# lucidrains/se3-transformer-pytorch

Hardware: NVIDIA H100
Metric: point-clouds/sec fwd (higher is better)
Workload: dtype f32

## Files before the change

### se3_transformer_pytorch_b200/csrc/zgemm.cu

```cuda
#include "common.cuh"
#include "tc_ptx.cuh"
#include <algorithm>
#include <cstdlib>
#include <type_traits>

namespace se3 {

constexpr int kZThreads = 384;
constexpr int kZMaxSeg = 16;
constexpr uint32_t kZWRingBytes = 196608;

template <int V>
using ic = std::integral_constant<int, V>;

template <class F, int... I>
__device__ __forceinline__ void static_for_seq(F&& f, std::integer_sequence<int, I...>) {
  (f(ic<I>()), ...);
}
template <int N, class F>
__device__ __forceinline__ void static_for(F&& f) {
  static_for_seq(f, std::make_integer_sequence<int, N>());
}

struct ZSeg {
  const float* U;
  const float* X;
  int Ci, ncomp, cplus, cminus, n_stage, pad;
};

struct ZParams {
  ZSeg seg[kZMaxSeg];
  int n_seg;
  const uint8_t* w_img;
  const float* sx;
  float* out;
  int64_t E;
  int64_t out_es;
  int comp_off[2];
  int n_mt, n_nt, S, flush_stages;
};

__device__ __forceinline__ void z_frag(const float (&v)[2][4], uint32_t (&hi)[4], uint32_t (&lo)[4]) {
  split_h2(v[0][0], v[0][1], hi[0], lo[0]);
  split_h2(v[1][0], v[1][1], hi[1], lo[1]);
  split_h2(v[0][2], v[0][3], hi[2], lo[2]);
  split_h2(v[1][2], v[1][3], hi[3], lo[3]);
}

template <int NR>
__device__ __forceinline__ void z_mma3(float (&d)[NR], const uint32_t (&hi)[4], const uint32_t (&lo)[4], uint64_t b_hi, uint64_t b_lo,
                                       uint32_t scale_d = 1) {
  if constexpr (NR == 64) {
    wgmma_rs_n128(d, hi, b_hi, scale_d);
    wgmma_rs_n128(d, lo, b_hi);
    wgmma_rs_n128(d, hi, b_lo);
  } else {
    wgmma_rs_n64(d, hi, b_hi, scale_d);
    wgmma_rs_n64(d, lo, b_hi);
    wgmma_rs_n64(d, hi, b_lo);
  }
}

template <int MODE, int N, int NC>
__global__ void __launch_bounds__(kZThreads, 1)
zgemm_kernel(const __grid_constant__ ZParams prm) {
  static_assert((MODE == 1 || MODE == 4) ? NC == 128 : NC == 64, "CTA width");
  static_assert(N % NC == 0 && (MODE == 1 || N == 128), "weight image tile");
  constexpr int NA = (MODE == 3) ? 3 : (MODE == 2) ? 2 : 1;
  constexpr int NO = (MODE == 2 || MODE == 3) ? 2 : 1;
  constexpr int NR = NC / 2;
  constexpr int NH = N / NC;
  constexpr uint32_t kImgStage = 2u * N * 128u;
  constexpr uint32_t kStageBytes = 2u * NC * 128u;
  constexpr int WS = (kZWRingBytes / kStageBytes > 8) ? 8 : (int)(kZWRingBytes / kStageBytes);

  extern __shared__ uint8_t smem_raw[];
  const uint32_t raw = smem_u32(smem_raw);
  const uint32_t base = (raw + 1023u) & ~1023u;
  const uint32_t sW = base;
  const uint32_t bar_w_full = sW + WS * kStageBytes;
  const uint32_t bar_w_empty = bar_w_full + 8 * WS;

  const int warp = __shfl_sync(0xffffffffu, (int)(threadIdx.x >> 5), 0), lane = threadIdx.x & 31;
  const int S = prm.S, FS = prm.flush_stages;
  const int n_ct = prm.n_nt * NH;
  const int ctile = (int)(blockIdx.x % n_ct);
  const int64_t mt = blockIdx.x / n_ct;
  const int nt = ctile / NH, hs = ctile % NH;

  if (threadIdx.x == 0) {
    for (int s = 0; s < WS; ++s) {
      mbar_init(bar_w_full + 8 * s, 1);
      mbar_init(bar_w_empty + 8 * s, 8);
    }
    asm volatile("fence.mbarrier_init.release.cluster;" ::: "memory");
  }
  __syncthreads();

  if (warp < 4) {
    asm volatile("setmaxnreg.dec.sync.aligned.u32 40;");
    if (warp == 0 && lane == 0) {
      const uint8_t* wsrc = prm.w_img + (size_t)nt * S * kImgStage + (size_t)hs * NC * 128u;
      for (int s = 0; s < S; ++s) {
        const int slot = s % WS;
        mbar_wait(bar_w_empty + 8 * slot, ((uint32_t)(s / WS) & 1u) ^ 1u);
        mbar_arrive_expect_tx(bar_w_full + 8 * slot, kStageBytes);
        bulk_g2s(sW + slot * kStageBytes, wsrc + (size_t)s * kImgStage, NC * 128u, bar_w_full + 8 * slot);
        bulk_g2s(sW + slot * kStageBytes + NC * 128u, wsrc + (size_t)s * kImgStage + N * 128u, NC * 128u, bar_w_full + 8 * slot);
      }
    }
    return;
  }
  asm volatile("setmaxnreg.inc.sync.aligned.u32 232;");
  const int ct = threadIdx.x - 128;
  const int r0 = (ct >> 7) * 64 + ((ct >> 5) & 3) * 16 + (lane >> 2);
  const int kq = 2 * (lane & 3);
  int64_t eg[2];
  bool live[2];
  float sxe[2];
#pragma unroll
  for (int rs = 0; rs < 2; ++rs) {
    eg[rs] = mt * SE3_TILE_E + r0 + 8 * rs;
    live[rs] = eg[rs] < prm.E;
    sxe[rs] = (live[rs] && MODE != 4) ? prm.sx[eg[rs]] : 1.f;
  }
  float D[NA][NR], acc[NO][NR];
#pragma unroll
  for (int a = 0; a < NA; ++a)
#pragma unroll
    for (int j = 0; j < NR; ++j) D[a][j] = 0.f;
#pragma unroll
  for (int a = 0; a < NO; ++a)
#pragma unroll
    for (int j = 0; j < NR; ++j) acc[a][j] = 0.f;
  int blk_start = 0;
  int fresh = 0;

  auto release = [&](int s) {
    __syncwarp();
    if (lane == 0) mbar_arrive(bar_w_empty + 8 * (s % WS));
  };
  auto drain_after = [&](int s) { return s + 1 == S || s + 1 - blk_start == FS; };
  auto drain = [&](int s) {
#pragma unroll
    for (int j = 0; j < NR; ++j) {
      if (MODE == 3) {
        acc[0][j] += D[0][j] - D[NA - 1][j];
        acc[1][j] += D[0][j] + D[NA > 1 ? 1 : 0][j];
      } else {
#pragma unroll
        for (int a = 0; a < NA; ++a) acc[a][j] += D[a][j];
      }
      if (MODE == 2 || MODE == 4)
#pragma unroll
        for (int a = 0; a < NA; ++a) D[a][j] = 0.f;
    }
    fresh = (1 << NA) - 1;
    blk_start = s + 1;
  };
  auto finish_stage = [&](int s) {
    wgmma_commit();
    wgmma_wait0();
    release(s);
    if (drain_after(s)) drain(s);
  };

  constexpr int ZR = (MODE == 3) ? 2 : 4;
  float u[2][4];
  auto zf = [&](const float (&y)[2], uint32_t (&hi)[4], uint32_t (&lo)[4]) {
    float v[2][4];
#pragma unroll
    for (int rs = 0; rs < 2; ++rs)
#pragma unroll
      for (int q = 0; q < 4; ++q) v[rs][q] = u[rs][q] * y[rs];
    z_frag(v, hi, lo);
  };
  auto chunk_mma = [&](auto cc, auto ac, int s, const float (&y)[2], uint64_t b_hi, uint64_t b_lo) {
    constexpr int C = decltype(cc)::value, A = decltype(ac)::value;
    wgmma_wait<ZR - 1>();
    if (C == ZR - 1 && s != blk_start) release(s - 1);
    uint32_t hi[4], lo[4];
    zf(y, hi, lo);
    wgmma_fence();
    z_mma3<NR>(D[A], hi, lo, b_hi + 2 * C, b_lo + 2 * C, ((fresh >> A) & 1) ^ 1);
    fresh &= ~(1 << A);
    wgmma_commit();
  };
  auto end_stage = [&](int s) {
    if (drain_after(s)) {
      wgmma_wait0();
      release(s);
      drain(s);
    }
  };
  auto wait_stage = [&](int s, uint64_t& b_hi, uint64_t& b_lo) {
    mbar_wait(bar_w_full + 8 * (s % WS), (uint32_t)(s / WS) & 1u);
    const uint32_t wb = sW + (uint32_t)(s % WS) * kStageBytes;
    b_hi = wg_desc_sw128(wb);
    b_lo = wg_desc_sw128(wb + NC * 128u);
  };

  if constexpr (MODE == 4) {
    const ZSeg& z = prm.seg[0];
    const int M = z.ncomp, Dn = z.Ci;
    int64_t node[2];
    int m[2];
    float sc[2];
    const float* xrow[2];
#pragma unroll
    for (int rs = 0; rs < 2; ++rs) {
      node[rs] = live[rs] ? eg[rs] / M : 0;
      m[rs] = live[rs] ? (int)(eg[rs] - node[rs] * M) : 0;
      sc[rs] = live[rs] ? prm.sx[node[rs]] : 1.f;
      xrow[rs] = z.X + ((size_t)node[rs] * Dn) * M + m[rs];
    }
    for (int s = 0; s < S; ++s) {
      float v[4][2][4];
#pragma unroll
      for (int c = 0; c < 4; ++c)
#pragma unroll
        for (int rs = 0; rs < 2; ++rs)
#pragma unroll
          for (int q = 0; q < 4; ++q) {
            const int d = 64 * s + 16 * c + kq + (q & 1) + 8 * (q >> 1);
            v[c][rs][q] = live[rs] ? __ldg(xrow[rs] + (size_t)d * M) * sc[rs] : 0.f;
          }
      uint64_t b_hi, b_lo;
      wait_stage(s, b_hi, b_lo);
      uint32_t hi[4][4], lo[4][4];
#pragma unroll
      for (int c = 0; c < 4; ++c) z_frag(v[c], hi[c], lo[c]);
      wgmma_fence();
#pragma unroll
      for (int c = 0; c < 4; ++c) z_mma3<NR>(D[0], hi[c], lo[c], b_hi + 2 * c, b_lo + 2 * c);
      finish_stage(s);
    }
#pragma unroll
    for (int rs = 0; rs < 2; ++rs) {
      if (!live[rs]) continue;
      const float inv = 1.f / sc[rs];
      const int64_t Eo = prm.out_es;
      const size_t o0 = (size_t)nt * N + (size_t)hs * NC + kq;
      float* dst = prm.out + ((size_t)node[rs] * Eo + o0) * M + m[rs];
      const float* res = z.U ? z.U + ((size_t)node[rs] * Eo + o0) * M + m[rs] : nullptr;
#pragma unroll
      for (int g = 0; g < NC / 8; ++g)
#pragma unroll
        for (int b = 0; b < 2; ++b) {
          const size_t o = (size_t)(8 * g + b) * M;
          dst[o] = acc[0][4 * g + 2 * rs + b] * inv + (res ? __ldg(res + o) : 0.f);
        }
    }
  } else {
    int s = 0;
    for (int sg = 0; sg < prm.n_seg; ++sg) {
      const ZSeg& z = prm.seg[sg];
      const int ns = z.n_stage;
      const size_t istride = (size_t)z.ncomp * 128;
      const float* xp = z.X + ((size_t)mt * z.Ci * z.ncomp + z.cplus) * 128 + r0;
      const float* xm = z.X + ((size_t)mt * z.Ci * z.ncomp + z.cminus) * 128 + r0;
#pragma unroll
      for (int rs = 0; rs < 2; ++rs) {
        const float* urow = z.U + (size_t)(live[rs] ? eg[rs] : 0) * 64;
#pragma unroll
        for (int q = 0; q < 4; ++q) u[rs][q] = live[rs] ? __ldg(urow + kq + (q & 1) + 8 * (q >> 1)) * sxe[rs] : 0.f;
      }
      if constexpr (MODE == 1) {
        float y[4][2];
#pragma unroll
        for (int c = 0; c < 4; ++c)
#pragma unroll
          for (int rs = 0; rs < 2; ++rs) y[c][rs] = __ldg(xp + c * istride + 8 * rs);
#pragma unroll 1
        for (int sl = 0; sl < ns; ++sl, ++s) {
          const float* xn = (sl + 1 < ns) ? xp + 4 * istride : xp;
          uint64_t b_hi, b_lo;
          wait_stage(s, b_hi, b_lo);
          static_for<4>([&](auto cc) {
            constexpr int C = decltype(cc)::value;
            chunk_mma(cc, ic<0>(), s, y[C], b_hi, b_lo);
#pragma unroll
            for (int rs = 0; rs < 2; ++rs) y[C][rs] = __ldg(xn + C * istride + 8 * rs);
          });
          end_stage(s);
          xp = xn;
        }
      } else if constexpr (MODE == 2) {
#pragma unroll 1
        for (int sl = 0; sl < ns; ++sl, ++s) {
          float yp[2][2], ym[2][2];
#pragma unroll
          for (int il = 0; il < 2; ++il)
#pragma unroll
            for (int rs = 0; rs < 2; ++rs) {
              const size_t o = (size_t)(2 * sl + il) * istride + 8 * rs;
              yp[il][rs] = __ldg(xp + o);
              ym[il][rs] = __ldg(xm + o);
            }
          uint64_t b_hi, b_lo;
          wait_stage(s, b_hi, b_lo);
          uint32_t hp[2][4], lp[2][4], hm[2][4], lm[2][4];
#pragma unroll
          for (int il = 0; il < 2; ++il) {
            zf(yp[il], hp[il], lp[il]);
            zf(ym[il], hm[il], lm[il]);
          }
          uint32_t hn[2][4], ln[2][4];
#pragma unroll
          for (int il = 0; il < 2; ++il)
#pragma unroll
            for (int q = 0; q < 4; ++q) { hn[il][q] = hm[il][q] ^ 0x80008000u; ln[il][q] = lm[il][q] ^ 0x80008000u; }
          wgmma_fence();
#pragma unroll
          for (int il = 0; il < 2; ++il) {
            const uint64_t ba_hi = b_hi + 2 * (2 * il), ba_lo = b_lo + 2 * (2 * il);
            const uint64_t bb_hi = b_hi + 2 * (2 * il + 1), bb_lo = b_lo + 2 * (2 * il + 1);
            z_mma3<NR>(D[0], hp[il], lp[il], ba_hi, ba_lo);
            z_mma3<NR>(D[0], hn[il], ln[il], bb_hi, bb_lo);
            z_mma3<NR>(D[NA - 1], hm[il], lm[il], ba_hi, ba_lo);
            z_mma3<NR>(D[NA - 1], hp[il], lp[il], bb_hi, bb_lo);
          }
          finish_stage(s);
        }
      } else {
        const int dmo = (z.cminus - z.cplus) * 128;
        float x[4][2][2];
#pragma unroll
        for (int j = 0; j < 4; ++j)
#pragma unroll
          for (int rs = 0; rs < 2; ++rs) {
            x[j][0][rs] = __ldg(xp + j * istride + 8 * rs);
            x[j][1][rs] = __ldg(xp + dmo + j * istride + 8 * rs);
          }
        const int np = ns / 3;
#pragma unroll 1
        for (int p = 0; p < np; ++p) {
          const size_t adv = (p + 1 < np) ? 4 * istride : 0;
          static_for<3>([&](auto tc) {
            uint64_t b_hi, b_lo;
            wait_stage(s, b_hi, b_lo);
            static_for<4>([&](auto cc) {
              constexpr int Q = 4 * decltype(tc)::value + decltype(cc)::value, J = Q / 3, T = Q % 3;
              float y[2];
#pragma unroll
              for (int rs = 0; rs < 2; ++rs) {
                const float cp = x[J][0][rs], dm = x[J][1][rs];
                y[rs] = (T == 0) ? cp : (T == 1) ? (dm - cp) : (cp + dm);
              }
              chunk_mma(cc, ic<T>(), s, y, b_hi, b_lo);
              if constexpr (T == 2) {
#pragma unroll
                for (int rs = 0; rs < 2; ++rs) {
                  x[J][0][rs] = __ldg(xp + adv + J * istride + 8 * rs);
                  x[J][1][rs] = __ldg(xp + adv + dmo + J * istride + 8 * rs);
                }
              }
            });
            end_stage(s);
            ++s;
          });
          xp += adv;
        }
      }
    }

#pragma unroll
    for (int rs = 0; rs < 2; ++rs) {
      if (!live[rs]) continue;
      const float inv = 1.f / sxe[rs];
#pragma unroll
      for (int a = 0; a < NO; ++a) {
        float* dst = prm.out + (size_t)eg[rs] * prm.out_es + prm.comp_off[a] + (size_t)nt * N + (size_t)hs * NC + kq;
#pragma unroll
        for (int g = 0; g < NC / 8; ++g)
          *reinterpret_cast<float2*>(dst + 8 * g) = make_float2(acc[a][4 * g + 2 * rs] * inv, acc[a][4 * g + 2 * rs + 1] * inv);
      }
    }
  }
}

__global__ void zpack_kernel(const float* __restrict__ Fp, int Kp, int col0, int Co, int CiF, int N, int S, int stage0, int n_stage,
                             int gauss, uint8_t* __restrict__ img) {
  const int nt = blockIdx.y, sl = blockIdx.x;
  uint8_t* dst = img + ((size_t)nt * S + stage0 + sl) * (2u * N * 128u);
  for (int t = threadIdx.x; t < N * 64; t += blockDim.x) {
    const int r = t >> 6, k = t & 63;
    const int o = nt * N + r;
    float w = 0.f;
    if (gauss) {
      const int q = sl * 4 + (k >> 4);
      const int ty = q % 3, i = q / 3;
      if (2 * i + 1 < CiF && o < Co) {
        const float wa = Fp[((size_t)o * CiF + 2 * i) * Kp + col0 + (k & 15)], wb = Fp[((size_t)o * CiF + 2 * i + 1) * Kp + col0 + (k & 15)];
        w = (ty == 0) ? wa + wb : (ty == 1) ? wa : wb;
      }
    } else {
      const int c = sl * 4 + (k >> 4);
      if (c < CiF && o < Co) w = Fp[((size_t)o * CiF + c) * Kp + col0 + (k & 15)];
    }
    const __half hi = __float2half_rn(w);
    const __half lo = __float2half_rn(w - __half2float(hi));
    const uint32_t off = (uint32_t)(r * 128 + (((k >> 3) ^ (r & 7)) << 4) + (k & 7) * 2);
    *reinterpret_cast<__half*>(dst + off) = hi;
    *reinterpret_cast<__half*>(dst + (size_t)N * 128 + off) = lo;
  }
}

template <int MODE, int N, int NC>
static int launch_z(const ZParams& prm, cudaStream_t s) {
  constexpr uint32_t kStageBytes = 2u * NC * 128u;
  constexpr int WS = (kZWRingBytes / kStageBytes > 8) ? 8 : (int)(kZWRingBytes / kStageBytes);
  const size_t smem = 1024 + (size_t)WS * kStageBytes + 256;
  auto kern = zgemm_kernel<MODE, N, NC>;
  SE3_CUDA_OK(cudaFuncSetAttribute(kern, cudaFuncAttributeMaxDynamicSharedMemorySize, (int)smem));
  const int64_t grid = (int64_t)prm.n_mt * prm.n_nt * (N / NC);
  SE3_REQUIRE(grid < 2147483647ll, "se3_zgemm: grid too large");
  kern<<<(unsigned)grid, kZThreads, smem, s>>>(prm);
  SE3_LAUNCH_OK();
  return SE3_OK;
}

static int z_env_int(const char* name, int dflt) {
  const char* v = getenv(name);
  return v ? atoi(v) : dflt;
}

}

extern "C" int se3_zgemm_tile_n(int Co, int mode) {
  if (Co <= 0 || Co % 128 != 0) return -1;
  if (mode == 2 || mode == 3 || mode == 4) return 128;
  if (mode != 1) return -1;
  return (Co % 256 == 0) ? 256 : 128;
}

extern "C" int64_t se3_zgemm_image_bytes(int Co, int mode, int total_stages) {
  const int N = se3_zgemm_tile_n(Co, mode);
  if (N < 0 || total_stages <= 0) return -1;
  return (int64_t)(Co / N) * total_stages * 2 * N * 128;
}

extern "C" int se3_zgemm_pack(const float* Fp, int Kp, int col0, int Co, int CiF, int mode, int total_stages, int stage0, void* image,
                              void* stream) {
  using namespace se3;
  const int N = se3_zgemm_tile_n(Co, mode);
  SE3_REQUIRE(N > 0, "se3_zgemm_pack: Co=%d must be a multiple of 128 (mode %d)", Co, mode);
  SE3_REQUIRE(Fp != nullptr && image != nullptr, "se3_zgemm_pack: null pointer");
  SE3_REQUIRE(Kp >= 16 && Kp % 16 == 0 && col0 >= 0 && col0 + 16 <= Kp, "se3_zgemm_pack: bad column range");
  SE3_REQUIRE(CiF > 0 && (mode == 1 || CiF % 2 == 0), "se3_zgemm_pack: bad sizes");
  const int n_stage = (mode == 3) ? 3 * (int)ceil_div(CiF / 2, 4) : (int)ceil_div(CiF, 4);
  SE3_REQUIRE(stage0 >= 0 && stage0 + n_stage <= total_stages, "se3_zgemm_pack: stage range outside the image");
  zpack_kernel<<<dim3((unsigned)n_stage, (unsigned)(Co / N)), 256, 0, as_stream(stream)>>>(Fp, Kp, col0, Co, CiF, N, total_stages, stage0, n_stage,
                                                                                         mode == 3 ? 1 : 0, reinterpret_cast<uint8_t*>(image));
  SE3_LAUNCH_OK();
  return SE3_OK;
}

extern "C" int se3_linear_tc_fwd(const float* x, const void* w_img, const float* res, const float* sx, int64_t nodes, int D, int Eo,
                                 int M, float* out, void* stream) {
  using namespace se3;
  SE3_REQUIRE(nodes > 0 && M >= 1 && M <= 11, "se3_linear_tc_fwd: bad sizes");
  SE3_REQUIRE(D > 0 && D % 64 == 0 && Eo > 0 && Eo % 128 == 0, "se3_linear_tc_fwd: D=%d must be a multiple of 64 and Eo=%d of 128", D, Eo);
  SE3_REQUIRE(x != nullptr && w_img != nullptr && sx != nullptr && out != nullptr, "se3_linear_tc_fwd: null pointer");
  ZParams prm;
  prm.n_seg = 1;
  prm.seg[0].U = res;
  prm.seg[0].X = x;
  prm.seg[0].Ci = D;
  prm.seg[0].ncomp = M;
  prm.seg[0].cplus = prm.seg[0].cminus = 0;
  prm.seg[0].n_stage = D / 64;
  prm.seg[0].pad = 0;
  prm.w_img = reinterpret_cast<const uint8_t*>(w_img);
  prm.sx = sx;
  prm.out = out;
  prm.E = nodes * M;
  prm.out_es = Eo;
  prm.comp_off[0] = prm.comp_off[1] = 0;
  prm.n_mt = (int)ceil_div(prm.E, SE3_TILE_E);
  prm.n_nt = Eo / 128;
  prm.S = D / 64;
  prm.flush_stages = std::max(1, z_env_int("SE3B200_Z_FLUSH", 8));
  return launch_z<4, 128, 128>(prm, as_stream(stream));
}

extern "C" int se3_zgemm_fwd(const se3_zseg* segs, int n_seg, const void* w_img, const float* sx, int64_t E, int Co, int mode,
                             float* out, int64_t out_edge_stride, int comp_off0, int comp_off1, int flush_stages, void* stream) {
  using namespace se3;
  const int N = se3_zgemm_tile_n(Co, mode);
  SE3_REQUIRE(N > 0 && mode != 4, "se3_zgemm_fwd: Co=%d must be a multiple of 128 and mode 1, 2 or 3 (got %d)", Co, mode);
  SE3_REQUIRE(E > 0 && n_seg >= 1 && n_seg <= kZMaxSeg, "se3_zgemm_fwd: bad sizes (1..%d segments)", kZMaxSeg);
  SE3_REQUIRE(segs != nullptr && w_img != nullptr && sx != nullptr && out != nullptr, "se3_zgemm_fwd: null pointer");
  SE3_REQUIRE(out_edge_stride >= Co && out_edge_stride % 4 == 0 && comp_off0 % 4 == 0 && comp_off1 % 4 == 0 &&
              (reinterpret_cast<uintptr_t>(out) & 15) == 0, "se3_zgemm_fwd: output rows must be 16-byte aligned");
  ZParams prm;
  prm.n_seg = n_seg;
  int S = 0;
  const int F = (mode == 1) ? 1 : 2;
  for (int i = 0; i < n_seg; ++i) {
    const se3_zseg& z = segs[i];
    SE3_REQUIRE(z.U != nullptr && z.X != nullptr && z.Ci > 0 && z.ncomp >= 1 && z.cplus >= 0 && z.cplus < z.ncomp &&
                z.cminus >= 0 && z.cminus < z.ncomp, "se3_zgemm_fwd: bad segment %d", i);
    SE3_REQUIRE((z.Ci * F) % 4 == 0 && (mode != 3 || z.Ci % 4 == 0), "se3_zgemm_fwd: C_in * F = %d must be a multiple of 4 (mode 3: C_in % 4 == 0)", z.Ci * F);
    prm.seg[i].U = z.U;
    prm.seg[i].X = z.X;
    prm.seg[i].Ci = z.Ci;
    prm.seg[i].ncomp = z.ncomp;
    prm.seg[i].cplus = z.cplus;
    prm.seg[i].cminus = z.cminus;
    prm.seg[i].n_stage = (mode == 3) ? 3 * (z.Ci / 4) : z.Ci * F / 4;
    prm.seg[i].pad = 0;
    S += prm.seg[i].n_stage;
  }
  prm.w_img = reinterpret_cast<const uint8_t*>(w_img);
  prm.sx = sx;
  prm.out = out;
  prm.E = E;
  prm.out_es = out_edge_stride;
  prm.comp_off[0] = comp_off0;
  prm.comp_off[1] = comp_off1;
  prm.n_mt = (int)ceil_div(E, SE3_TILE_E);
  prm.n_nt = Co / N;
  prm.S = S;
  prm.flush_stages = std::max(1, flush_stages > 0 ? flush_stages
                                                     : z_env_int("SE3B200_Z_FLUSH", mode == 3 ? 24 : 8) * std::max(1, z_env_int("SE3B200_Z_FLUSH_MULT", 1)));
  cudaStream_t s = as_stream(stream);
  if (mode == 3) return launch_z<3, 128, 64>(prm, s);
  if (mode == 2) return launch_z<2, 128, 64>(prm, s);
  return N == 256 ? launch_z<1, 256, 128>(prm, s) : launch_z<1, 128, 128>(prm, s);
}
```

Baseline: 1.924.

## Spill MODE 3 accumulators to shared memory and hoist drain checks out of stage loops

For the three-way MODE 3 z-GEMM, the running output accumulators move from registers into a per-thread slot in shared memory. The drain step reads, adds and writes them back as float4, which frees registers so the wgmma pipeline depth ZR can go from 2 to 3 (it drops from 4 to 3 for the other modes). The stage loops in MODE 1 and 3 are split into runs of flush_stages length, so the drain check runs once per run instead of once per stage. The flush length is clamped to S and rounded to a multiple of 3 for MODE 3. This adds shared-memory traffic at each drain, costs extra shared memory, and lowers the pipeline depth for MODE 1.

```diff
diff --git a/se3_transformer_pytorch_b200/csrc/zgemm.cu b/se3_transformer_pytorch_b200/csrc/zgemm.cu
--- a/se3_transformer_pytorch_b200/csrc/zgemm.cu
+++ b/se3_transformer_pytorch_b200/csrc/zgemm.cu
@@ -73,12 +73,14 @@
   constexpr uint32_t kImgStage = 2u * N * 128u;
   constexpr uint32_t kStageBytes = 2u * NC * 128u;
   constexpr int WS = (kZWRingBytes / kStageBytes > 8) ? 8 : (int)(kZWRingBytes / kStageBytes);
+  constexpr uint32_t kAccBytes = (MODE == 3) ? NO * NR * 256u * 4u : 0u;
 
   extern __shared__ uint8_t smem_raw[];
   const uint32_t raw = smem_u32(smem_raw);
   const uint32_t base = (raw + 1023u) & ~1023u;
   const uint32_t sW = base;
-  const uint32_t bar_w_full = sW + WS * kStageBytes;
+  float4* const sacc = reinterpret_cast<float4*>(smem_raw + (base - raw) + WS * kStageBytes);
+  const uint32_t bar_w_full = sW + WS * kStageBytes + kAccBytes;
   const uint32_t bar_w_empty = bar_w_full + 8 * WS;
 
   const int warp = __shfl_sync(0xffffffffu, (int)(threadIdx.x >> 5), 0), lane = threadIdx.x & 31;
@@ -133,6 +135,10 @@
   for (int a = 0; a < NO; ++a)
 #pragma unroll
     for (int j = 0; j < NR; ++j) acc[a][j] = 0.f;
+  if constexpr (MODE == 3) {
+#pragma unroll
+    for (int g = 0; g < NO * NR / 4; ++g) sacc[g * 256 + ct] = make_float4(0.f, 0.f, 0.f, 0.f);
+  }
   int blk_start = 0;
   int fresh = 0;
 
@@ -142,18 +148,28 @@
   };
   auto drain_after = [&](int s) { return s + 1 == S || s + 1 - blk_start == FS; };
   auto drain = [&](int s) {
-#pragma unroll
-    for (int j = 0; j < NR; ++j) {
-      if (MODE == 3) {
-        acc[0][j] += D[0][j] - D[NA - 1][j];
-        acc[1][j] += D[0][j] + D[NA > 1 ? 1 : 0][j];
-      } else {
+    if constexpr (MODE == 3) {
+#pragma unroll
+      for (int g = 0; g < NR / 4; ++g) {
+        const float4 p = sacc[g * 256 + ct], m = sacc[(NR / 4 + g) * 256 + ct];
+        float sp[4] = {p.x, p.y, p.z, p.w}, sm[4] = {m.x, m.y, m.z, m.w};
+#pragma unroll
+        for (int q = 0; q < 4; ++q) {
+          sp[q] += D[0][4 * g + q] - D[2][4 * g + q];
+          sm[q] += D[0][4 * g + q] + D[1][4 * g + q];
+        }
+        sacc[g * 256 + ct] = make_float4(sp[0], sp[1], sp[2], sp[3]);
+        sacc[(NR / 4 + g) * 256 + ct] = make_float4(sm[0], sm[1], sm[2], sm[3]);
+      }
+    } else {
+#pragma unroll
+      for (int j = 0; j < NR; ++j) {
 #pragma unroll
         for (int a = 0; a < NA; ++a) acc[a][j] += D[a][j];
-      }
-      if (MODE == 2 || MODE == 4)
-#pragma unroll
-        for (int a = 0; a < NA; ++a) D[a][j] = 0.f;
+        if (MODE == 2 || MODE == 4)
+#pragma unroll
+          for (int a = 0; a < NA; ++a) D[a][j] = 0.f;
+      }
     }
     fresh = (1 << NA) - 1;
     blk_start = s + 1;
@@ -165,7 +181,7 @@
     if (drain_after(s)) drain(s);
   };
 
-  constexpr int ZR = (MODE == 3) ? 2 : 4;
+  constexpr int ZR = 3;
   float u[2][4];
   auto zf = [&](const float (&y)[2], uint32_t (&hi)[4], uint32_t (&lo)[4]) {
     float v[2][4];
@@ -186,7 +202,7 @@
     fresh &= ~(1 << A);
     wgmma_commit();
   };
-  auto end_stage = [&](int s) {
+  auto end_run = [&](int s) {
     if (drain_after(s)) {
       wgmma_wait0();
       release(s);
@@ -271,19 +287,22 @@
         for (int c = 0; c < 4; ++c)
 #pragma unroll
           for (int rs = 0; rs < 2; ++rs) y[c][rs] = __ldg(xp + c * istride + 8 * rs);
+        for (int sl = 0; sl < ns;) {
+          const int run_end = min(ns, sl + (blk_start + FS - s));
 #pragma unroll 1
-        for (int sl = 0; sl < ns; ++sl, ++s) {
-          const float* xn = (sl + 1 < ns) ? xp + 4 * istride : xp;
-          uint64_t b_hi, b_lo;
-          wait_stage(s, b_hi, b_lo);
-          static_for<4>([&](auto cc) {
-            constexpr int C = decltype(cc)::value;
-            chunk_mma(cc, ic<0>(), s, y[C], b_hi, b_lo);
-#pragma unroll
-            for (int rs = 0; rs < 2; ++rs) y[C][rs] = __ldg(xn + C * istride + 8 * rs);
-          });
-          end_stage(s);
-          xp = xn;
+          for (; sl < run_end; ++sl, ++s) {
+            const float* xn = (sl + 1 < ns) ? xp + 4 * istride : xp;
+            uint64_t b_hi, b_lo;
+            wait_stage(s, b_hi, b_lo);
+            static_for<4>([&](auto cc) {
+              constexpr int C = decltype(cc)::value;
+              chunk_mma(cc, ic<0>(), s, y[C], b_hi, b_lo);
+#pragma unroll
+              for (int rs = 0; rs < 2; ++rs) y[C][rs] = __ldg(xn + C * istride + 8 * rs);
+            });
+            xp = xn;
+          }
+          end_run(s - 1);
         }
       } else if constexpr (MODE == 2) {
 #pragma unroll 1
@@ -333,37 +352,52 @@
             x[j][1][rs] = __ldg(xp + dmo + j * istride + 8 * rs);
           }
         const int np = ns / 3;
+        for (int p = 0; p < np;) {
+          const int run_end = min(np, p + (blk_start + FS - s) / 3);
 #pragma unroll 1
-        for (int p = 0; p < np; ++p) {
-          const size_t adv = (p + 1 < np) ? 4 * istride : 0;
-          static_for<3>([&](auto tc) {
-            uint64_t b_hi, b_lo;
-            wait_stage(s, b_hi, b_lo);
-            static_for<4>([&](auto cc) {
-              constexpr int Q = 4 * decltype(tc)::value + decltype(cc)::value, J = Q / 3, T = Q % 3;
-              float y[2];
-#pragma unroll
-              for (int rs = 0; rs < 2; ++rs) {
-                const float cp = x[J][0][rs], dm = x[J][1][rs];
-                y[rs] = (T == 0) ? cp : (T == 1) ? (dm - cp) : (cp + dm);
-              }
-              chunk_mma(cc, ic<T>(), s, y, b_hi, b_lo);
-              if constexpr (T == 2) {
+          for (; p < run_end; ++p) {
+            const size_t adv = (p + 1 < np) ? 4 * istride : 0;
+            static_for<3>([&](auto tc) {
+              uint64_t b_hi, b_lo;
+              wait_stage(s, b_hi, b_lo);
+              static_for<4>([&](auto cc) {
+                constexpr int Q = 4 * decltype(tc)::value + decltype(cc)::value, J = Q / 3, T = Q % 3;
+                float y[2];
 #pragma unroll
                 for (int rs = 0; rs < 2; ++rs) {
-                  x[J][0][rs] = __ldg(xp + adv + J * istride + 8 * rs);
-                  x[J][1][rs] = __ldg(xp + adv + dmo + J * istride + 8 * rs);
+                  const float cp = x[J][0][rs], dm = x[J][1][rs];
+                  y[rs] = (T == 0) ? cp : (T == 1) ? (dm - cp) : (cp + dm);
                 }
-              }
+                chunk_mma(cc, ic<T>(), s, y, b_hi, b_lo);
+                if constexpr (T == 2) {
+#pragma unroll
+                  for (int rs = 0; rs < 2; ++rs) {
+                    x[J][0][rs] = __ldg(xp + adv + J * istride + 8 * rs);
+                    x[J][1][rs] = __ldg(xp + adv + dmo + J * istride + 8 * rs);
+                  }
+                }
+              });
+              ++s;
             });
-            end_stage(s);
-            ++s;
-          });
-          xp += adv;
+            xp += adv;
+          }
+          end_run(s - 1);
         }
       }
     }
 
+    if constexpr (MODE == 3) {
+#pragma unroll
+      for (int a = 0; a < NO; ++a)
+#pragma unroll
+        for (int g = 0; g < NR / 4; ++g) {
+          const float4 v = sacc[(a * NR / 4 + g) * 256 + ct];
+          acc[a][4 * g] = v.x;
+          acc[a][4 * g + 1] = v.y;
+          acc[a][4 * g + 2] = v.z;
+          acc[a][4 * g + 3] = v.w;
+        }
+    }
 #pragma unroll
     for (int rs = 0; rs < 2; ++rs) {
       if (!live[rs]) continue;
@@ -410,7 +444,8 @@
 static int launch_z(const ZParams& prm, cudaStream_t s) {
   constexpr uint32_t kStageBytes = 2u * NC * 128u;
   constexpr int WS = (kZWRingBytes / kStageBytes > 8) ? 8 : (int)(kZWRingBytes / kStageBytes);
-  const size_t smem = 1024 + (size_t)WS * kStageBytes + 256;
+  constexpr uint32_t kAccBytes = (MODE == 3) ? 2u * (NC / 2) * 256u * 4u : 0u;
+  const size_t smem = 1024 + (size_t)WS * kStageBytes + kAccBytes + 256;
   auto kern = zgemm_kernel<MODE, N, NC>;
   SE3_CUDA_OK(cudaFuncSetAttribute(kern, cudaFuncAttributeMaxDynamicSharedMemorySize, (int)smem));
   const int64_t grid = (int64_t)prm.n_mt * prm.n_nt * (N / NC);
@@ -522,8 +557,10 @@
   prm.n_mt = (int)ceil_div(E, SE3_TILE_E);
   prm.n_nt = Co / N;
   prm.S = S;
-  prm.flush_stages = std::max(1, flush_stages > 0 ? flush_stages
-                                                     : z_env_int("SE3B200_Z_FLUSH", mode == 3 ? 24 : 8) * std::max(1, z_env_int("SE3B200_Z_FLUSH_MULT", 1)));
+  int fs = std::min(S, std::max(1, flush_stages > 0 ? flush_stages
+                                                    : z_env_int("SE3B200_Z_FLUSH", mode == 3 ? 24 : 8) * std::max(1, z_env_int("SE3B200_Z_FLUSH_MULT", 1))));
+  if (mode == 3) fs = (fs + 2) / 3 * 3;
+  prm.flush_stages = fs;
   cudaStream_t s = as_stream(stream);
   if (mode == 3) return launch_z<3, 128, 64>(prm, s);
   if (mode == 2) return launch_z<2, 128, 64>(prm, s);
```

New measurement: 1.977 (median of 6 runs). +2.8%, better.
